# ECP-WarpX/WarpX

Hardware: AMD Instinct MI355X
Metric: particle_steps_per_s (higher is better)
Workload: dtype f64; 1 GPU; 3D uniform_plasma 256x256x256, 8 ppc, Yee FDTD, order-3 shape, esirkepov, boris, filter on; cells_per_gpu=16777216, particles_per_gpu=134217728, n_ranks=1, ranks_per_gpu=1, sort_interval=2, single_precision_comms=False, preroll_steps=40, overlap_halo=False, momentum_synchronisation=outside the timed region (the K steps are consecutive steps of one longer run)

## Files before the change

include/warpx_amd.h:

```cpp
#ifndef WARPX_AMD_H_
#define WARPX_AMD_H_

#include <stdint.h>

#ifdef __cplusplus
extern "C" {
#endif

typedef enum wxa_status {
    WXA_OK = 0,
    WXA_ERR_INVALID_ARG = -1,
    WXA_ERR_HIP = -2,
    WXA_ERR_UNSUPPORTED = -3,
    WXA_ERR_NOMEM = -4,
    WXA_ERR_COMM = -5
} wxa_status;

enum { WXA_PUSHER_BORIS = 0, WXA_PUSHER_VAY = 1, WXA_PUSHER_HC = 2,
       WXA_PUSHER_BORIS_RR = 3 };
enum { WXA_DEPOSIT_ESIRKEPOV = 0, WXA_DEPOSIT_DIRECT = 1 };
enum { WXA_DT_FULL = 0, WXA_DT_FIRST_HALF = 1, WXA_DT_SECOND_HALF = 2 };

typedef struct wxa_field_view {
    double* p;
// ... 168 lines not shown
                                    const int32_t sm_lo[3], const int32_t sm_hi[3], void* stream);

#define WXA_PBOUNDARY_DEFAULT    0
#define WXA_PBOUNDARY_ABSORBING  1
#define WXA_PBOUNDARY_REFLECTING 2
#define WXA_PBOUNDARY_PERIODIC   3

wxa_status wxa_apply_particle_boundaries(const wxa_particle_view* p, const double prob_lo[3],
                                         const double prob_hi[3], const int32_t bc_lo[3],
                                         const int32_t bc_hi[3], int64_t* n_lost,
                                         wxa_workspace* ws, void* stream);

wxa_status wxa_apply_pec_j(const wxa_field_view J[3], const int32_t dom_lo[3],
                           const int32_t dom_hi[3], const int32_t pec_lo[3],
                           const int32_t pec_hi[3], void* stream);

wxa_status wxa_apply_pec_rho(const wxa_field_view* rho, const int32_t dom_lo[3],
                             const int32_t dom_hi[3], const int32_t pec_lo[3],
                             const int32_t pec_hi[3], void* stream);


wxa_status wxa_filter_bilinear(const wxa_field_view* src, const wxa_field_view* dst,
                               void* stream);

wxa_status wxa_filter_stencil(const wxa_field_view* src, const wxa_field_view* dst, const double* s0, int32_t n0,
                              const double* s1, int32_t n1, const double* s2, int32_t n2, void* stream);

#define WXA_NCI_EX_EY_BZ 0
#define WXA_NCI_BX_BY_EZ 1
wxa_status wxa_nci_godfrey_stencil(double cdtodz, int32_t nodal_gather, int32_t coeff_set, double stencil_z[5]);

wxa_status wxa_fill_boundary_periodic(const wxa_field_view* f, const int ng[3],
                                      const int periodic[3], void* stream);

wxa_status wxa_fill_boundary_periodic_multi(const wxa_field_view* f, int32_t nf, const int ng[3],
                                            const int periodic[3], void* stream);

wxa_status wxa_sync_nodal_periodic(const wxa_field_view* f, const int periodic[3], void* stream);

wxa_status wxa_sum_boundary_periodic(const wxa_field_view* f, const int src_ng[3],
                                     const int periodic[3], void* stream);

wxa_status wxa_sum_boundary_periodic_multi(const wxa_field_view* f, int32_t nf, const int src_ng[3],
                                           const int periodic[3], void* stream);

wxa_status wxa_pack_box(const wxa_field_view* f, const int32_t blo[3], const int32_t bhi[3],
// ... 204 lines not shown
```

warpx_amd/_capi.py:

```python
from __future__ import annotations

import ctypes as C
import os

_HERE = os.path.dirname(os.path.abspath(__file__))
PRODUCT_LIB = os.path.join(_HERE, "libwarpx_amd.so")


class FieldView(C.Structure):
    _fields_ = [
        ("p", C.c_void_p),
        ("lo", C.c_int32 * 3),
        ("n", C.c_int32 * 3),
        ("ng", C.c_int32 * 3),
        ("stag", C.c_int32 * 3),
        ("jstride", C.c_int64),
        ("kstride", C.c_int64),
    ]


class ParticleView(C.Structure):
    _fields_ = [
        ("x", C.c_void_p), ("y", C.c_void_p), ("z", C.c_void_p), ("w", C.c_void_p),
        ("ux", C.c_void_p), ("uy", C.c_void_p), ("uz", C.c_void_p),
# ... 194 lines not shown
    "sim_get_field": (C.c_int, [C.c_void_p, C.c_char_p, _PFV]),
    "sim_get_particles": (C.c_int, [C.c_void_p, C.c_int32, _PPV]),
    "sim_get_timers": (C.c_int, [C.c_void_p, C.c_double * 8, C.c_int64 * 8, C.c_int]),
    "sim_enable_timers": (C.c_int, [C.c_void_p, C.c_int]),
    "sim_compute_rho": (C.c_int, [C.c_void_p]),
    "sim_halo_overlap": (C.c_int32, [C.c_void_p]),
    "sim_set_moving_window": (C.c_int, [C.c_void_p, C.POINTER(MovingWindow)]),
    "sim_set_injection": (C.c_int, [C.c_void_p, C.c_int32, C.POINTER(PlasmaInjector), C.c_int, C.c_int]),
    "sim_set_external_particle_fields": (C.c_int, [C.c_void_p, C.c_int32, _D3, _D3]),
    "sim_set_radiation_reaction": (C.c_int, [C.c_void_p, C.c_int32, C.c_int32]),
    "sim_add_laser": (C.c_int, [C.c_void_p, C.POINTER(LaserAntenna)]),
    "sim_add_btd": (C.c_int, [C.c_void_p, C.c_int32, C.c_double, C.c_int32, C.c_int32]),
    "sim_btd_num_particles": (C.c_int, [C.c_void_p, C.c_int32, C.c_int32, C.POINTER(C.c_int64)]),
    "sim_btd_particles": (C.c_int, [C.c_void_p, C.c_int32, C.c_int32, C.POINTER(C.c_double)]),
    "sim_btd_info": (C.c_int, [C.c_void_p, C.c_int32, C.POINTER(C.c_int32), C.POINTER(C.c_double), C.POINTER(C.c_double),
                              C.POINTER(C.c_int32), C.POINTER(C.c_int32)]),
    "sim_btd_data": (C.c_int, [C.c_void_p, C.c_int32, C.c_int32, C.POINTER(C.c_double)]),
    "sim_add_reduced_diag": (C.c_int, [C.c_void_p, C.c_char_p, C.c_char_p, C.c_char_p, C.c_char_p]),
    "sim_reduced_diag_data": (C.c_int, [C.c_void_p, C.c_char_p, C.c_int32, C.POINTER(C.c_double), C.c_int32,
                                       C.POINTER(C.c_int32)]),
}

_PRODUCT_SIGS = {
    "fill_boundary_periodic_multi": (C.c_int, [_PFV, C.c_int32, _I3, _I3, C.c_void_p]),
    "sum_boundary_periodic_multi": (C.c_int, [_PFV, C.c_int32, _I3, _I3, C.c_void_p]),
    "workspace_set_external_particle_fields": (C.c_int, [C.c_void_p, _D3, _D3]),
    "workspace_set_repeated_plasma_lens": (C.c_int, [C.c_void_p, C.POINTER(RepeatedPlasmaLens)]),
    "workspace_set_time": (C.c_int, [C.c_void_p, C.c_double]),
    "workspace_create": (C.c_int, [C.POINTER(C.c_void_p)]),
    "workspace_destroy": (None, [C.c_void_p]),
    "last_error": (C.c_char_p, []),
    "sort_particles_by_cell": (C.c_int, [_PPV, _PPV, _D3, _D3, _I32_3, _I32_3, C.c_void_p, C.c_void_p]),
    "gather_push_ws": (C.c_int, [_PPV, _FV3, _FV3, _PGG, C.c_double, C.c_double, C.c_double,
                                 C.c_int, C.c_int, C.c_int, C.c_int, C.c_void_p, C.c_void_p]),
    "add_plasma": (C.c_int, [_PPV, C.POINTER(PlasmaInjector), _D3, _I32_3, _D3, _D3, _D3,
                             C.POINTER(InjectedMomentum), C.POINTER(C.c_int64), C.c_void_p, C.c_void_p]),
    "gather_push_part": (C.c_int, [_PPV, _FV3, _FV3, _PGG, C.c_double, C.c_double, C.c_double, C.c_int, C.c_int,
                                   C.c_int, C.c_void_p, C.c_int, C.c_void_p]),
    "partition_particles": (C.c_int, [_PPV, _PPV, C.c_int, C.c_double, C.c_double,
                                      C.POINTER(C.c_int64), C.c_void_p, C.c_void_p]),
    "wrap_and_classify": (C.c_int, [_PPV, C.c_int64, C.c_int64, _D3, _D3, _I3, _D3, _D3, _I3, C.c_void_p,
                                    C.c_int64, C.POINTER(C.c_int64), C.c_void_p, C.c_void_p]),
    "wrap_and_classify_dest": (C.c_int, [_PPV, C.c_int64, C.c_int64, _D3, _D3, _I3, _D3, _D3, _I3, C.c_void_p,
                                         C.c_int64, C.POINTER(C.c_int64), C.c_void_p, C.c_void_p]),
    "pack_leavers": (C.c_int, [_PPV, C.c_void_p, C.c_int64, C.c_void_p, C.c_int64, C.c_int64, C.c_int, _D3, _D3,
                               C.c_void_p]),
# ... 176 lines not shown
```

warpx_amd/csrc/fields.hip:

```cpp
#include "common.hpp"

#include <algorithm>
#include <climits>
#include <cstdlib>

namespace wxa {

template <int TW_, int TJ_, int KC_, int NT_, int BATCH_ = 0>
struct StencilCfg {
    static constexpr int TW = TW_, TI = 64 * TW_, TJ = TJ_, KC = KC_, NT = NT_, BATCH = BATCH_;
};

struct TileGrid {
    int nti, ntj, ntk;
    long ntiles;
};

template <class CFG>
static TileGrid make_tiles_cfg(const Box3& ub) {
    TileGrid t;
    t.nti = (ub.hi[0] - ub.lo[0] + CFG::TI - 1) / CFG::TI;
    t.ntj = (ub.hi[1] - ub.lo[1] + CFG::TJ - 1) / CFG::TJ;
    t.ntk = (ub.hi[2] - ub.lo[2] + CFG::KC - 1) / CFG::KC;
    t.ntiles = (long)t.nti * t.ntj * t.ntk;
// ... 438 lines not shown
    DevF f[WXA_MULTI_MAX];
    BoxN lo[WXA_MULTI_MAX], hi[WXA_MULTI_MAX];
    int shift[WXA_MULTI_MAX];
};
__global__ void __launch_bounds__(256)
shift_copy_sides_multi_kernel(SideCopySet a, int d) {
    const int c = blockIdx.y;
    const DevF f = a.f[c];
    const BoxN box_lo = a.lo[c], box_hi = a.hi[c];
    const int s0 = d == 0 ? a.shift[c] : 0, s1 = d == 1 ? a.shift[c] : 0, s2 = d == 2 ? a.shift[c] : 0;
    const long half = (long)box_lo.n[0] * box_lo.n[1] * box_lo.n[2];
    for (long t = (long)blockIdx.x * blockDim.x + threadIdx.x; t < 2 * half; t += (long)gridDim.x * blockDim.x) {
        const bool hi = t >= half;
        const long u = hi ? t - half : t;
        const BoxN& box = hi ? box_hi : box_lo;
        const int sg = hi ? -1 : 1;
        const int aa = (int)(u % box.n[0]);
        const int bb = (int)((u / box.n[0]) % box.n[1]);
        const int cc = (int)(u / ((long)box.n[0] * box.n[1]));
        const int i = box.lo[0] + aa, j = box.lo[1] + bb, k = box.lo[2] + cc;
        f.p[f.off(i, j, k)] = f.p[f.off(i + sg * s0, j + sg * s1, k + sg * s2)];
    }
}
struct PeriodicSumSet {
    DevF f[WXA_MULTI_MAX];
    int nc[WXA_MULTI_MAX], s0[WXA_MULTI_MAX], s1[WXA_MULTI_MAX];
};
__global__ void __launch_bounds__(256)
sum_periodic_multi_kernel(PeriodicSumSet a, int d) {
    const int c = blockIdx.y;
    const DevF f = a.f[c];
    const int nc = a.nc[c], s0 = a.s0[c], s1 = a.s1[c];
    const int lo[3] = {f.lo0, f.lo1, f.lo2};
    const int n[3] = {f.n0, f.n1, f.n2};
    const long st[3] = {1, f.js, f.ks};
    const int da = d == 0 ? 1 : 0, db = d == 2 ? 1 : 2;
    const int nr = n[d] - nc;
    if (nr <= 0) return;
    const long total = (long)n[da] * nr * n[db];
    for (long t = (long)blockIdx.x * blockDim.x + threadIdx.x; t < total; t += (long)gridDim.x * blockDim.x) {
        int aa, r, b;
        if (d == 0) {
            r = (int)(t % nr); aa = (int)((t / nr) % n[da]); b = (int)(t / ((long)nr * n[da]));
        } else {
            aa = (int)(t % n[da]); r = (int)((t / n[da]) % nr); b = (int)(t / ((long)n[da] * nr));
        }
// ... 176 lines not shown
            double* b = &By(i, j, k);
            __builtin_nontemporal_store(__builtin_nontemporal_load(b) + (dt * ckc_up_x(ez, c.x, i, j, k) - dt * ckc_up_z(ex, c.z, i, j, k)), b);
        }
        if (pz && k >= bbz.lo[2] && k < bbz.hi[2]) {
            double* b = &Bz(i, j, k);
            __builtin_nontemporal_store(__builtin_nontemporal_load(b) + (dt * ckc_up_y(ex, c.y, i, j, k) - dt * ckc_up_x(ey, c.x, i, j, k)), b);
        }
        if constexpr (CFG::PIPE) {
            if (more) {
                ckc_put_plane<CFG>(ring[0] + ((k + 2) & 3) * PLANE, rx, tid);
                ckc_put_plane<CFG>(ring[1] + ((k + 2) & 3) * PLANE, ry, tid);
                ckc_put_plane<CFG>(ring[2] + ((k + 2) & 3) * PLANE, rz, tid);
            }
        }
        if constexpr (CFG::PIPE == 2) {
#pragma unroll
            for (int n = 0; n < CFG::PER; ++n) { rx[n] = qx[n]; ry[n] = qy[n]; rz[n] = qz[n]; }
        }
    }
}

using CkcProduction = CkcCfg<4, 16, 2>;
using FilterCfg = CkcCfg<8, 16, 1>;

struct FilterStencils {
    static constexpr int MAXLEN = 8;
    double s[3][MAXLEN];
    int n[3];
};
__global__ void __launch_bounds__(256)
filter_stencil_kernel(DevF src, DevF dst, FilterStencils fs) {
    const long total = (long)src.n0 * src.n1 * src.n2;
    for (long t = (long)blockIdx.x * blockDim.x + threadIdx.x; t < total; t += (long)gridDim.x * blockDim.x) {
        const int i = src.lo0 + (int)(t % src.n0);
        const int j = src.lo1 + (int)((t / src.n0) % src.n1);
        const int k = src.lo2 + (int)(t / ((long)src.n0 * src.n1));
        auto zp = [&](int ii, int jj, int kk) -> double {
            return (ii >= src.lo0 && ii < src.lo0 + src.n0 && jj >= src.lo1 && jj < src.lo1 + src.n1 && kk >= src.lo2 &&
                    kk < src.lo2 + src.n2) ? src.p[src.off(ii, jj, kk)] : 0.0;
        };
        double d = 0.0;
        for (int i2 = 0; i2 < fs.n[2]; ++i2)
            for (int i1 = 0; i1 < fs.n[1]; ++i1)
                for (int i0 = 0; i0 < fs.n[0]; ++i0) {
                    const double sss = fs.s[0][i0] * fs.s[1][i1] * fs.s[2][i2];
                    d += sss * (zp(i - i0, j - i1, k - i2) + zp(i + i0, j - i1, k - i2) + zp(i - i0, j + i1, k - i2) +
// ... 16 lines not shown
    const int k0 = src.lo2 + (int)(t / columns) * KC, k1 = min(k0 + KC, src.lo2 + src.n2);
    auto zp = [&](int kk) -> double { return (kk >= src.lo2 && kk < src.lo2 + src.n2) ? src.p[src.off(i, j, kk)] : 0.0; };
    double w[2 * N2 - 1];
#pragma unroll
    for (int m = 0; m < 2 * N2 - 1; ++m) w[m] = zp(k0 - (N2 - 1) + m);
    double sss[N2];
#pragma unroll
    for (int i2 = 0; i2 < N2; ++i2) sss[i2] = fs.s[0][0] * fs.s[1][0] * fs.s[2][i2];
    for (int k = k0; k < k1; ++k) {
        const double next = zp(k + N2);
        double d = 0.0;
#pragma unroll
        for (int i2 = 0; i2 < N2; ++i2) {
            const double a = w[N2 - 1 - i2], b = w[N2 - 1 + i2];
            d += sss[i2] * (a + a + a + a + b + b + b + b);
        }
        dst.p[dst.off(i, j, k)] = d;
#pragma unroll
        for (int m = 0; m + 1 < 2 * N2 - 1; ++m) w[m] = w[m + 1];
        w[2 * N2 - 2] = next;
    }
}

template <class CFG>
__global__ void __launch_bounds__(CFG::NT)
filter_bilinear_kernel(DevF src, DevF dst, TileGrid tg) {
    constexpr int PLANE = CFG::PLANE;
    __shared__ double ring[4 * PLANE];
    const long tile = xcd_tile_id(blockIdx.x, tg.ntiles);
    if (tile >= tg.ntiles) return;
    const int ti = (int)(tile % tg.nti), tj = (int)((tile / tg.nti) % tg.ntj), tk = (int)(tile / ((long)tg.nti * tg.ntj));
    const int i0 = src.lo0 + ti * CFG::TI, j0 = src.lo1 + tj * CFG::TJ, k0 = src.lo2 + tk * CFG::KC;
    const int hi0 = src.lo0 + src.n0, hi1 = src.lo1 + src.n1, hi2 = src.lo2 + src.n2;
    const int k1 = min(k0 + CFG::KC, hi2);
    const int tid = (int)(threadIdx.y * CFG::TI + threadIdx.x);
    const int i = i0 + (int)threadIdx.x, j = j0 + (int)threadIdx.y;
    double r[CFG::PER];
    for (int k = k0 - 1; k <= k0 + 1; ++k) {
        ckc_fetch_plane<CFG>(r, src, i0, j0, k, tid);
        ckc_put_plane<CFG>(ring + (k & 3) * PLANE, r, tid);
    }
    const CkcRing<CFG> in{ring, i0, j0};
    const bool active = i < hi0 && j < hi1;
    for (int k = k0; k < k1; ++k) {
        __syncthreads();
        const bool more = k + 2 <= k1;
        if (more) ckc_fetch_plane<CFG>(r, src, i0, j0, k + 2, tid);
        if (active) {
            auto tap = [&](int di, int dj, int dk) -> double { return in(i + di, j + dj, k + dk); };
            double d = 0.0;
#pragma unroll
            for (int i2 = 0; i2 < 2; ++i2)
#pragma unroll
                for (int i1 = 0; i1 < 2; ++i1)
#pragma unroll
                    for (int i0_ = 0; i0_ < 2; ++i0_) {
                        const double sss = 0.25 * 0.25 * 0.25;
                        d += sss * (tap(-i0_, -i1, -i2) + tap(+i0_, -i1, -i2) + tap(-i0_, +i1, -i2) +
                                    tap(+i0_, +i1, -i2) + tap(-i0_, -i1, +i2) + tap(+i0_, -i1, +i2) +
                                    tap(-i0_, +i1, +i2) + tap(+i0_, +i1, +i2));
                    }
            dst.p[dst.off(i, j, k)] = d;
        }
        if (more) ckc_put_plane<CFG>(ring + ((k + 2) & 3) * PLANE, r, tid);
    }
}

static inline int grid_for(long total, int block = 256, int cap = 256 * 16) {
    long g = (total + block - 1) / block;
    if (g < 1) g = 1;
    if (g > cap) g = cap;
    return (int)g;
}

static bool box_inside(const wxa_field_view& v, const int32_t blo[3], const int32_t bhi[3]) {
    for (int d = 0; d < 3; ++d)
        if (blo[d] < v.lo[d] || bhi[d] > v.lo[d] + v.n[d] || bhi[d] < blo[d]) return false;
    return true;
}

}

using namespace wxa;

extern "C" {

wxa_status wxa_evolve_b(const wxa_field_view E[3], const wxa_field_view B[3], double dt,
                        const double dinv[3], void* stream) {
// ... 181 lines not shown
    const Box3 bx = valid_box(E[0]), by = valid_box(E[1]), bz = valid_box(E[2]);
    for (int c = 0; c < 3; ++c) {
        const Box3 bj = valid_box(J[c]);
        const Box3 be = valid_box(E[c]);
        for (int d = 0; d < 3; ++d)
            WXA_REQUIRE(bj.lo[d] == be.lo[d] && bj.hi[d] == be.hi[d], "J and E valid boxes differ");
    }
    Box3 ub;
    for (int d = 0; d < 3; ++d) {
        ub.lo[d] = std::min(bx.lo[d], std::min(by.lo[d], bz.lo[d]));
        ub.hi[d] = std::max(bx.hi[d], std::max(by.hi[d], bz.hi[d]));
    }
    using CFG = StProduction;
    const TileGrid tg = make_tiles_cfg<CFG>(ub);
    if (tg.ntiles > 0)
        hipLaunchKernelGGL((evolve_e_kernel<CFG>), dim3((unsigned)xcd_grid_size(tg.ntiles)), dim3(CFG::TI, CFG::TJ), 0,
                           (hipStream_t)stream, make_devf(E[0]), make_devf(E[1]), make_devf(E[2]), make_devf(B[0]),
                           make_devf(B[1]), make_devf(B[2]), make_devf(J[0]), make_devf(J[1]), make_devf(J[2]), ub, bx, by, bz,
                           tg, dt, dinv[0], dinv[1], dinv[2]);
    WXA_LAUNCH_CHECK();
    return WXA_OK;
}

wxa_status wxa_filter_bilinear(const wxa_field_view* src, const wxa_field_view* dst, void* stream) {
    WXA_REQUIRE(src && dst && view_ok(*src) && view_ok(*dst), "bad field view");
    WXA_REQUIRE(src->p != dst->p, "src and dst must not alias");
    for (int d = 0; d < 3; ++d)
        WXA_REQUIRE(src->lo[d] == dst->lo[d] && src->n[d] == dst->n[d], "src/dst boxes differ");
    TileGrid tg;
    tg.nti = (src->n[0] + FilterCfg::TI - 1) / FilterCfg::TI;
    tg.ntj = (src->n[1] + FilterCfg::TJ - 1) / FilterCfg::TJ;
    tg.ntk = (src->n[2] + FilterCfg::KC - 1) / FilterCfg::KC;
    tg.ntiles = (long)tg.nti * tg.ntj * tg.ntk;
    hipLaunchKernelGGL(filter_bilinear_kernel<FilterCfg>, dim3((unsigned)xcd_grid_size(tg.ntiles)),
                       dim3(FilterCfg::TI, FilterCfg::TJ), 0, (hipStream_t)stream, make_devf(*src), make_devf(*dst), tg);
    WXA_LAUNCH_CHECK();
    return WXA_OK;
}

wxa_status wxa_filter_stencil(const wxa_field_view* src, const wxa_field_view* dst, const double* s0, int32_t n0,
                              const double* s1, int32_t n1, const double* s2, int32_t n2, void* stream) {
    WXA_REQUIRE(src && dst && view_ok(*src) && view_ok(*dst) && s0 && s1 && s2, "bad argument");
    WXA_REQUIRE(src->p != dst->p, "src and dst must not alias");
    WXA_REQUIRE(n0 >= 1 && n0 <= FilterStencils::MAXLEN && n1 >= 1 && n1 <= FilterStencils::MAXLEN && n2 >= 1 &&
                n2 <= FilterStencils::MAXLEN, "stencil length");
    for (int d = 0; d < 3; ++d)
        WXA_REQUIRE(src->lo[d] == dst->lo[d] && src->n[d] == dst->n[d], "src/dst boxes differ");
    FilterStencils fs;
    fs.n[0] = n0; fs.n[1] = n1; fs.n[2] = n2;
    for (int a = 0; a < FilterStencils::MAXLEN; ++a) {
        fs.s[0][a] = a < n0 ? s0[a] : 0.0; fs.s[1][a] = a < n1 ? s1[a] : 0.0; fs.s[2][a] = a < n2 ? s2[a] : 0.0;
    }
    const long total = (long)src->n[0] * src->n[1] * src->n[2];
    if (total == 0) return WXA_OK;
    if (n0 == 1 && n1 == 1 && n2 == 5) {
        constexpr int KC = 32;
        const long lanes = (long)src->n[0] * src->n[1] * ((src->n[2] + KC - 1) / KC);
        hipLaunchKernelGGL((filter_stencil_z_kernel<5, KC>), dim3((unsigned)((lanes + 255) / 256)), dim3(256), 0,
                           (hipStream_t)stream, make_devf(*src), make_devf(*dst), fs);
        WXA_LAUNCH_CHECK();
// ... 28 lines not shown
        sh[d] = nc;
        const long total = 2 * (long)blo.n[0] * blo.n[1] * blo.n[2];
        if (total > 0)
            hipLaunchKernelGGL(shift_copy_sides_kernel, dim3(grid_for(total)), dim3(256), 0, (hipStream_t)stream, df,
                               blo, bhi, sh[0], sh[1], sh[2]);
        lo[d] = v0 - ng[d];
        hi[d] = v1 + ng[d];
    }
    WXA_LAUNCH_CHECK();
    return WXA_OK;
}

wxa_status wxa_fill_boundary_periodic_multi(const wxa_field_view* f, int32_t nf, const int ng[3], const int periodic[3],
                                            void* stream) {
    WXA_REQUIRE(f && ng && periodic && nf >= 1 && nf <= WXA_MULTI_MAX, "bad argument");
    int lo[WXA_MULTI_MAX][3], hi[WXA_MULTI_MAX][3];
    for (int c = 0; c < nf; ++c) {
        WXA_REQUIRE(view_ok(f[c]), "bad field view");
        for (int d = 0; d < 3; ++d) {
            WXA_REQUIRE(ng[d] <= f[c].ng[d], "ng exceeds allocated guards");
            lo[c][d] = f[c].lo[d] + f[c].ng[d];
            hi[c][d] = f[c].lo[d] + f[c].n[d] - f[c].ng[d];
        }
    }
    for (int d = 0; d < 3; ++d) {
        if (!periodic[d] || ng[d] <= 0) continue;
        SideCopySet a;
        long most = 0;
        for (int c = 0; c < nf; ++c) {
            const int nc = f[c].n[d] - 2 * f[c].ng[d] - f[c].stag[d];
            WXA_REQUIRE(ng[d] <= nc, "guard depth exceeds the period");
            const int v0 = f[c].lo[d] + f[c].ng[d], v1 = f[c].lo[d] + f[c].n[d] - f[c].ng[d];
            a.f[c] = make_devf(f[c]);
            for (int e = 0; e < 3; ++e) { a.lo[c].lo[e] = a.hi[c].lo[e] = lo[c][e]; a.lo[c].n[e] = a.hi[c].n[e] = hi[c][e] - lo[c][e]; }
            a.lo[c].lo[d] = v0 - ng[d]; a.hi[c].lo[d] = v1;
            a.lo[c].n[d] = a.hi[c].n[d] = ng[d];
            a.shift[c] = nc;
            most = std::max(most, 2 * (long)a.lo[c].n[0] * a.lo[c].n[1] * a.lo[c].n[2]);
            lo[c][d] = v0 - ng[d];
            hi[c][d] = v1 + ng[d];
        }
        for (int c = nf; c < WXA_MULTI_MAX; ++c) { a.f[c] = a.f[0]; a.lo[c] = a.lo[0]; a.hi[c] = a.hi[0]; a.shift[c] = 0; }
        if (most > 0)
            hipLaunchKernelGGL(shift_copy_sides_multi_kernel, dim3(grid_for(most), (unsigned)nf), dim3(256), 0,
                               (hipStream_t)stream, a, d);
    }
// ... 304 lines not shown
```

warpx_amd/csrc/host/BrickComm.hpp:

```cpp
#ifndef WXA_HOST_BRICKCOMM_HPP_
#define WXA_HOST_BRICKCOMM_HPP_

#include "amrex_shim.hpp"

namespace wxa::host {

struct DeviceBuffer {
    const Backend* be = nullptr;
    void* p = nullptr;
    size_t cap = 0;
    void reserve(size_t bytes) {
        if (bytes <= cap) return;
        if (p) be->dfree(p);
        cap = bytes + bytes / 4 + 1024;
        p = be->dmalloc(cap);
        if (!p) throw std::runtime_error("DeviceBuffer: allocation failed");
    }
    ~DeviceBuffer() { if (p) be->dfree(p); }
};

struct Slabs {
    int32_t smlo[3], smhi[3], splo[3], sphi[3], rplo[3], rphi[3], rmlo[3], rmhi[3];
};

// ... 40 lines not shown
    void set_periodic(const int periodic[3]) {
        for (int d = 0; d < 3; ++d) m_periodic[d] = periodic[d] != 0;
    }
    bool periodic(int d) const { return m_periodic[d]; }
    bool has_neighbor(int d, int side) const {
        return m_periodic[d] || (side == 0 ? m_coord[d] > 0 : m_coord[d] < m_nb[d] - 1);
    }
    bool exchanges(int d) const { return m_nb[d] > 1; }
    int rank_of(const int c[3]) const { return c[0] + m_nb[0] * (c[1] + m_nb[1] * c[2]); }
    int neighbor(int d, int side) const {
        if (!has_neighbor(d, side)) return -1;
        int c[3] = {m_coord[0], m_coord[1], m_coord[2]};
        c[d] = (c[d] + (side ? 1 : -1) + m_nb[d]) % m_nb[d];
        return rank_of(c);
    }
    const int* nbricks() const { return m_nb; }
    const int* coord() const { return m_coord; }

    bool domain_face(int d, int side) const { return side == 0 ? m_coord[d] == 0 : m_coord[d] == m_nb[d] - 1; }
    bool reference_corners() const { return m_reference_corners; }
    void FillBoundary(const std::vector<amrex::MultiFab*>& mfs, const amrex::IntVect& ng, bool nodal_sync,
                      void* stream) {
        const size_t nf = mfs.size();
        std::vector<std::array<int, 3>> lo(nf), hi(nf);
        for (size_t c = 0; c < nf; ++c) {
            const wxa_field_view& f = mfs[c]->view();
            for (int d = 0; d < 3; ++d) {
                if (ng[d] > f.ng[d]) throw std::runtime_error("FillBoundary: ng exceeds allocated guard cells");
                lo[c][d] = f.lo[d] + f.ng[d];
                hi[c][d] = f.lo[d] + f.n[d] - f.ng[d];
                if (!m_periodic[d] && !reference_corners()) { lo[c][d] = f.lo[d]; hi[c][d] = f.lo[d] + f.n[d]; }
            }
        }
        for (int d = 0; d < 3; ++d) {
            if (!m_periodic[d] && !exchanges(d)) continue;
            if (self_periodic(d)) {
                if (!nodal_sync && ng[d] > 0 && m_be->fill_boundary_periodic_multi && nf >= 2 && nf <= 6) {
                    wxa_field_view v[6];
                    for (size_t c = 0; c < nf; ++c) v[c] = transverse_view(mfs[c]->view(), d, lo[c].data(), hi[c].data());
                    int per[3] = {0, 0, 0}, g[3] = {0, 0, 0};
                    per[d] = 1; g[d] = ng[d];
                    check(m_be->fill_boundary_periodic_multi(v, (int32_t)nf, g, per, stream));
                } else {
                    for (size_t c = 0; c < nf; ++c) {
                        const wxa_field_view& f = mfs[c]->view();
                        if (nodal_sync && f.stag[d]) self_op(f, d, 0, lo[c].data(), hi[c].data(), true, stream);
// ... 319 lines not shown
```

warpx_amd/csrc/host/WarpX.hpp:

```cpp
#ifndef WXA_HOST_WARPX_HPP_
#define WXA_HOST_WARPX_HPP_

#include <chrono>
#include <functional>

#include "BTDiagnostics.hpp"
#include "NCIGodfreyFilter.hpp"
#include "ReducedDiags.hpp"
#include "WarpXParticleContainer.hpp"

namespace wxa::host {

struct guardCellManager {
    amrex::IntVect ng_alloc_EB, ng_alloc_J, ng_depos_J, ng_FieldSolver, ng_FieldGather, ng_UpdateAux;

    void Init(const amrex::Real dt, const std::array<amrex::Real, 3>& dx, const int nox, const bool use_filter,
              const amrex::IntVect& bilinear_filter_stencil_length, const bool do_fdtd_nci_corr = false,
              const int nci_corr_stencil = 0, const bool safe_guard_cells = false) {
        constexpr double c = 299'792'458.;
        for (int d = 0; d < 3; ++d) {
            const int ng_tmp = nox;
            ng_alloc_EB[d] = (ng_tmp % 2) ? ng_tmp + 1 : ng_tmp;
            if (d == 2 && do_fdtd_nci_corr) {
                const int ng = ng_tmp + nci_corr_stencil;
// ... 438 lines not shown
        m_overlap = true;
    }
    bool halo_overlap() const { return m_overlap; }
    void order_streams(void* waiting_stream, int ev, void* recorded_stream) {
        if (!m_halo_events[ev]) return;
        m_be->event_record(m_halo_events[ev], recorded_stream);
        m_be->stream_wait_event(waiting_stream, m_halo_events[ev]);
    }

    void PushParticlesandDeposit(amrex::Real a_cur_time, bool skip_current = false,
                                 PushType push_type = PushType::Explicit) {
        if (m_eb_fill_in_flight) {
            mypc->PushInterior(m_fields, dt[0]);
            order_streams(m_ctx.stream, 3, m_comm_stream);
            m_eb_fill_in_flight = false;
        }
        mypc->Evolve(m_fields, 0, "current_fp", a_cur_time, dt[0], DtType::Full, skip_current, push_type);
    }

    void SyncCurrentAndRho() {
        PhaseTimer t(&m_ctx, kSyncCurrent);
        using warpx::fields::FieldType;
        auto J = m_fields.get_alldirs(FieldType::current_fp, 0);
        if (use_filter)
            for (int idim = 0; idim < 3; ++idim) ApplyFilterJ(J, 0, idim);
        if (m_overlap) {
            order_streams(m_comm_stream, 0, m_ctx.stream);
            SumBoundaryJ(J, 0, m_comm_stream);
            return;
        }
        SumBoundaryJ(J, 0);
        ApplyJfieldBoundary(0, J[0], J[1], J[2], PatchType::fine);
    }

    void ApplyJfieldBoundary(int , amrex::MultiFab* Jx, amrex::MultiFab* Jy, amrex::MultiFab* Jz,
                             PatchType ) {
        if (!m_pec_here) return;
        const wxa_field_view Jv[3] = {Jx->view(), Jy->view(), Jz->view()};
        if (m_be->apply_pec_j(Jv, m_dom_lo, m_dom_hi, m_pec_lo, m_pec_hi, m_ctx.stream) != 0)
            throw std::runtime_error("apply_pec_j failed");
    }

    amrex::MultiFab& ComputeRho() {
        if (!m_rho) {
            amrex::IntVect ng_rho;
            for (int d = 0; d < 3; ++d)
                ng_rho[d] = m_ctx.nox + 1 + static_cast<int>(std::ceil(299'792'458. * dt[0] / m_ctx.dx[d]));
            m_rho = std::make_unique<amrex::MultiFab>(m_be, m_ctx.brick_box, amrex::IntVect(1), ng_rho);
// ... 32 lines not shown
                    total += (size_t)(sl.hi[0] - sl.lo[0]) * (size_t)(sl.hi[1] - sl.lo[1]) * (size_t)(sl.hi[2] - sl.lo[2]);
                    slabs.push_back(sl);
                }
            }
        }
        if (total) {
            m_pec_rho_keep.be = m_be;
            m_pec_rho_keep.reserve(sizeof(double) * total);
            for (const Slab& sl : slabs)
                check(m_be->pack_box(&v, sl.lo, sl.hi, static_cast<double*>(m_pec_rho_keep.p) + sl.at, m_ctx.stream), "pack_box");
        }
        if (m_be->apply_pec_rho(&v, m_dom_lo, m_dom_hi, m_pec_lo, m_pec_hi, m_ctx.stream) != 0)
            throw std::runtime_error("apply_pec_rho failed");
        for (const Slab& sl : slabs)
            check(m_be->unpack_box(&v, sl.lo, sl.hi, static_cast<const double*>(m_pec_rho_keep.p) + sl.at,  0,
                                   m_ctx.stream), "unpack_box");
    }

    void ApplyFilterJ(const ablastr::fields::VectorField& current, int , int idim) {
        amrex::MultiFab& J = *current[idim];
        amrex::MultiFab& tmp = *m_filter_tmp[idim];
        check(m_be->filter_bilinear(&J.view(), &tmp.view(), m_ctx.stream), "filter_bilinear");
        J.swap_storage(tmp);
    }

    void SumBoundaryJ(const ablastr::fields::VectorField& current, int lev) { SumBoundaryJ(current, lev, m_ctx.stream); }
    void SumBoundaryJ(const ablastr::fields::VectorField& current, int , void* stream) {
        amrex::IntVect ng_depos_J = guard_cells.ng_depos_J;
        if (use_filter) ng_depos_J = ng_depos_J + amrex::IntVect(2) - amrex::IntVect(1);
        ng_depos_J = amrex::min(ng_depos_J, current[0]->nGrowVect());
        m_comm->SumBoundary({current[0], current[1], current[2]}, ng_depos_J, safe_guard_cells,
                            stream);
    }

    void DryComm(int reps, double ms[4]) {
        using warpx::fields::FieldType;
        reps = std::min(std::max(reps, 1), 64);
        auto J = m_fields.get_alldirs(FieldType::current_fp, 0);
        DeviceBuffer saved[3];
        for (int c = 0; c < 3; ++c) {
            const wxa_field_view v = J[c]->view();
            const size_t bytes = sizeof(double) * (size_t)v.kstride * (size_t)v.n[2];
            saved[c].be = m_be;
            saved[c].reserve(bytes);
            m_be->memcpy_async(saved[c].p, v.p, bytes, m_ctx.stream);
        }
// ... 200 lines not shown
```

warpx_amd/csrc/host/backend.hpp:

```cpp
#ifndef WXA_HOST_BACKEND_HPP_
#define WXA_HOST_BACKEND_HPP_

#include <cstddef>
#include <cstdint>

#include "../../../include/warpx_amd.h"

struct wxa_expr;

namespace wxa::host {

struct Backend {
    const char* name;
    int (*evolve_b)(const wxa_field_view*, const wxa_field_view*, double, const double*, void*);
    int (*evolve_e)(const wxa_field_view*, const wxa_field_view*, const wxa_field_view*, double,
                    const double*, void*);
    int (*evolve_b_guard_layer)(const wxa_field_view*, const wxa_field_view*, double, const double*, const int32_t* grow,
                                void*);
    void (*ckc_stencil_coefficients)(const double* cell_size, double* cx, double* cy, double* cz);
    double (*ckc_max_dt)(const double* cell_size);
    int (*evolve_b_ckc)(const wxa_field_view*, const wxa_field_view*, double, const double* cx, const double* cy,
                        const double* cz, void*);
    int (*ws_set_external_eb)(void* ws, const double* E, const double* B);
    int (*ws_set_repeated_plasma_lens)(void* ws, const wxa_repeated_plasma_lens*) = nullptr;
// ... 13 lines not shown
    int (*add_plasma_profile)(const wxa_particle_view* dst, const wxa_plasma_injector*, const double* corner,
                              const int32_t* ncells, const double* dx, const double* brick_lo, const double* brick_hi,
                              const wxa_injected_momentum* momentum, const wxa_expr* density,
                              const wxa_expr* const* momentum_exprs, double density_min, double density_max,
                              int64_t* n_added, void* ws, void*) = nullptr;
    int (*ws_set_injection_profile)(void* ws, const wxa_expr* density, const wxa_expr* const* momentum) = nullptr;
    const char* (*last_error)() = nullptr;
    int (*deposit_charge)(const wxa_particle_view*, const wxa_field_view*, const wxa_grid_geom*, double, int, void*);
    int (*apply_pec_e)(const wxa_field_view*, const int32_t* dom_lo, const int32_t* dom_hi, const int32_t* pec_lo,
                       const int32_t* pec_hi, const int32_t* ng, void*);
    int (*apply_pec_b)(const wxa_field_view*, const int32_t* dom_lo, const int32_t* dom_hi, const int32_t* pec_lo,
                       const int32_t* pec_hi, const int32_t* ng, void*);
    int (*apply_pec_j)(const wxa_field_view*, const int32_t* dom_lo, const int32_t* dom_hi, const int32_t* pec_lo,
                       const int32_t* pec_hi, void*);
    int (*apply_pec_rho)(const wxa_field_view*, const int32_t* dom_lo, const int32_t* dom_hi, const int32_t* pec_lo,
                         const int32_t* pec_hi, void*);
    int (*apply_silver_mueller)(const wxa_field_view* E, const wxa_field_view* B, double dt, const double* dinv,
                                const int32_t* dom_lo, const int32_t* dom_hi, const int32_t* sm_lo, const int32_t* sm_hi,
                                void*) = nullptr;
    int (*shift_field_window)(const wxa_field_view*, double* tmp, int32_t dir, int32_t num_shift, const int* periodic,
                              void*);
    int (*laser_push)(const wxa_particle_view*, const wxa_laser_push_params*, double t, double dt, void*);
    int (*filter_bilinear)(const wxa_field_view*, const wxa_field_view*, void*);
    int (*btd_select_particles)(const wxa_particle_view*, const double* const old6[6], double z_boost, double z_boost_old,
                                double t_boost, double dt, double t_lab, double gamma_boost, double* out, int64_t capacity,
                                int64_t* n_selected, void* stream) = nullptr;
    int (*reduce_field)(const wxa_field_view*, const int32_t* lo, const int32_t* hi, double* sum_sq, double* max_abs,
                        void* stream) = nullptr;
    int (*reduce_particles)(const wxa_particle_view*, double mass, int32_t photon, double* out6, void* stream) = nullptr;
    int (*filter_stencil)(const wxa_field_view*, const wxa_field_view*, const double* s0, int32_t n0, const double* s1,
                          int32_t n1, const double* s2, int32_t n2, void*) = nullptr;
    int (*fill_boundary_periodic)(const wxa_field_view*, const int*, const int*, void*);
    int (*sync_nodal_periodic)(const wxa_field_view*, const int*, void*);
    int (*sum_boundary_periodic)(const wxa_field_view*, const int*, const int*, void*);
    int (*fill_boundary_periodic_multi)(const wxa_field_view*, int32_t, const int*, const int*, void*) = nullptr;
    int (*sum_boundary_periodic_multi)(const wxa_field_view*, int32_t, const int*, const int*, void*) = nullptr;
    int (*pack_box)(const wxa_field_view*, const int32_t*, const int32_t*, double*, void*);
    int (*unpack_box)(const wxa_field_view*, const int32_t*, const int32_t*, const double*, int, void*);
    int (*pack_box_f32)(const wxa_field_view*, const int32_t*, const int32_t*, float*, void*) = nullptr;
    int (*unpack_box_f32)(const wxa_field_view*, const int32_t*, const int32_t*, const float*, int, void*) = nullptr;
    int (*field_set_zero)(const wxa_field_view*, void*);
    int (*field_set_zero_multi)(const wxa_field_view*, int32_t, void*) = nullptr;
    int (*enforce_periodic)(const wxa_particle_view*, const double*, const double*, const int*, void*);
    int (*enforce_periodic_sorted)(const wxa_particle_view*, const double*, const double*, const int*, void* ws, int32_t,
                                   void*) = nullptr;
    int (*sort_particles_by_cell)(const wxa_particle_view*, const wxa_particle_view*, const double*,
// ... 42 lines not shown
```

warpx_amd/csrc/host/warpx_host.hip:

```cpp
#include <hip/hip_runtime.h>

#include "../common.hpp"
#include "WarpXInputs.hpp"

namespace {

using wxa::host::Backend;

void* hip_dmalloc(size_t bytes) {
    void* p = nullptr;
    if (hipMalloc(&p, bytes ? bytes : 8) != hipSuccess) {
        wxa::set_last_error("hipMalloc of %zu bytes failed", bytes);
        return nullptr;
    }
    return p;
}
void hip_dfree(void* p) { if (p) (void)hipFree(p); }
int hip_memset_async(void* p, int v, size_t n, void* st) {
    return hipMemsetAsync(p, v, n, (hipStream_t)st) == hipSuccess ? 0 : WXA_ERR_HIP;
}
int hip_memcpy_async(void* d, const void* s, size_t n, void* st) {
    if (n == 0) return 0;
    return hipMemcpyAsync(d, s, n, hipMemcpyDeviceToDevice, (hipStream_t)st) == hipSuccess ? 0 : WXA_ERR_HIP;
}
// ... 64 lines not shown
                           const wxa_grid_geom* g, double q, double m, double dt, int o, int ga, int pu, int move,
                           void* ws, void* st) -> int {
            return wxa_gather_push_ws(p, E, B, g, q, m, dt, o, ga, pu, move, static_cast<wxa_workspace*>(ws), st); };
        b.gather_push_part = [](const wxa_particle_view* p, const wxa_field_view* E, const wxa_field_view* B,
                                const wxa_grid_geom* g, double q, double m, double dt, int o, int ga, int pu, void* ws,
                                int part, void* st) -> int {
            return wxa_gather_push_part(p, E, B, g, q, m, dt, o, ga, pu, static_cast<wxa_workspace*>(ws), part, st); };
        b.add_plasma = [](const wxa_particle_view* dst, const wxa_plasma_injector* inj, const double* corner,
                          const int32_t* nc, const double* dx, const double* blo, const double* bhi,
                          const wxa_injected_momentum* u, int64_t* n, void* ws, void* st) -> int {
            return wxa_add_plasma(dst, inj, corner, nc, dx, blo, bhi, u, n, static_cast<wxa_workspace*>(ws), st); };
        b.add_plasma_profile = [](const wxa_particle_view* dst, const wxa_plasma_injector* inj, const double* corner,
                                  const int32_t* nc, const double* dx, const double* blo, const double* bhi,
                                  const wxa_injected_momentum* u, const wxa_expr* dens, const wxa_expr* const* mom,
                                  double dmin, double dmax, int64_t* n, void* ws, void* st) -> int {
            return wxa_add_plasma_profile(dst, inj, corner, nc, dx, blo, bhi, u, dens, mom, dmin, dmax, n,
                                          static_cast<wxa_workspace*>(ws), st); };
        b.ws_set_injection_profile = [](void* ws, const wxa_expr* dens, const wxa_expr* const* mom) -> int {
            return wxa_workspace_set_injection_profile(static_cast<wxa_workspace*>(ws), dens, mom); };
        b.last_error = wxa_last_error;
        b.deposit_current = k_deposit;
        b.filter_bilinear = [](const wxa_field_view* s, const wxa_field_view* d, void* st) -> int {
            return wxa_filter_bilinear(s, d, st); };
        b.btd_select_particles = [](const wxa_particle_view* p, const double* const o[6], double zb, double zbo, double tb,
                                    double dt, double tl, double g, double* out, int64_t cap, int64_t* n, void* st) -> int {
            return wxa_btd_select_particles(p, o, zb, zbo, tb, dt, tl, g, out, cap, n, st); };
        b.reduce_field = [](const wxa_field_view* f, const int32_t* lo, const int32_t* hi, double* ss, double* mx,
                            void* st) -> int { return wxa_reduce_field(f, lo, hi, ss, mx, st); };
        b.reduce_particles = [](const wxa_particle_view* p, double m, int32_t photon, double* out, void* st) -> int {
            return wxa_reduce_particles(p, m, photon, out, st); };
        b.filter_stencil = [](const wxa_field_view* s, const wxa_field_view* d, const double* s0, int32_t n0,
                              const double* s1, int32_t n1, const double* s2, int32_t n2, void* st) -> int {
            return wxa_filter_stencil(s, d, s0, n0, s1, n1, s2, n2, st); };
        b.fill_boundary_periodic = [](const wxa_field_view* f, const int* ng, const int* per, void* st) -> int {
            return wxa_fill_boundary_periodic(f, ng, per, st); };
        b.sync_nodal_periodic = [](const wxa_field_view* f, const int* per, void* st) -> int {
            return wxa_sync_nodal_periodic(f, per, st); };
        b.sum_boundary_periodic = [](const wxa_field_view* f, const int* ng, const int* per, void* st) -> int {
            return wxa_sum_boundary_periodic(f, ng, per, st); };
        b.fill_boundary_periodic_multi = [](const wxa_field_view* f, int32_t nf, const int* ng, const int* per, void* st) -> int {
            return wxa_fill_boundary_periodic_multi(f, nf, ng, per, st); };
        b.sum_boundary_periodic_multi = [](const wxa_field_view* f, int32_t nf, const int* ng, const int* per, void* st) -> int {
            return wxa_sum_boundary_periodic_multi(f, nf, ng, per, st); };
        b.pack_box = [](const wxa_field_view* f, const int32_t* lo, const int32_t* hi, double* buf, void* st) -> int {
            return wxa_pack_box(f, lo, hi, buf, st); };
        b.unpack_box = [](const wxa_field_view* f, const int32_t* lo, const int32_t* hi, const double* buf, int mode,
// ... 125 lines not shown
```

Before: 11.16 billion particle-steps/s.

## Batch J filter into one launch, deepen prefetch, fuse periodic guard fill

Merges the three per-component bilinear current filters into a single multi-field kernel launch indexed by blockIdx.y. The filter now prefetches AHEAD planes into registers instead of one, to hide global load latency. Separately, periodic guard-cell fill across two or more directions becomes a single shell-copy kernel instead of sequential per-direction passes. This cuts launch count and serialization, at the cost of more registers per thread and an extra host-side fast path in FillBoundary.

```diff
diff --git a/include/warpx_amd.h b/include/warpx_amd.h
--- a/include/warpx_amd.h
+++ b/include/warpx_amd.h
@@ -214,6 +214,8 @@
 
 wxa_status wxa_filter_bilinear(const wxa_field_view* src, const wxa_field_view* dst,
                                void* stream);
+
+wxa_status wxa_filter_bilinear_multi(const wxa_field_view* src, const wxa_field_view* dst, int32_t nf, void* stream);
 
 wxa_status wxa_filter_stencil(const wxa_field_view* src, const wxa_field_view* dst, const double* s0, int32_t n0,
                               const double* s1, int32_t n1, const double* s2, int32_t n2, void* stream);
diff --git a/warpx_amd/_capi.py b/warpx_amd/_capi.py
--- a/warpx_amd/_capi.py
+++ b/warpx_amd/_capi.py
@@ -240,6 +240,7 @@
 }
 
 _PRODUCT_SIGS = {
+    "filter_bilinear_multi": (C.c_int, [_PFV, _PFV, C.c_int32, C.c_void_p]),
     "fill_boundary_periodic_multi": (C.c_int, [_PFV, C.c_int32, _I3, _I3, C.c_void_p]),
     "sum_boundary_periodic_multi": (C.c_int, [_PFV, C.c_int32, _I3, _I3, C.c_void_p]),
     "workspace_set_external_particle_fields": (C.c_int, [C.c_void_p, _D3, _D3]),
diff --git a/warpx_amd/csrc/fields.hip b/warpx_amd/csrc/fields.hip
--- a/warpx_amd/csrc/fields.hip
+++ b/warpx_amd/csrc/fields.hip
@@ -484,6 +484,41 @@
         f.p[f.off(i, j, k)] = f.p[f.off(i + sg * s0, j + sg * s1, k + sg * s2)];
     }
 }
+struct GuardShellSet {
+    DevF f[WXA_MULTI_MAX];
+    int v0[WXA_MULTI_MAX][3], v1[WXA_MULTI_MAX][3];
+    int nc[WXA_MULTI_MAX][3];
+    int g[3];
+};
+__global__ void __launch_bounds__(256)
+fill_guard_shell_multi_kernel(GuardShellSet a) {
+    const int c = blockIdx.y / 3, d = blockIdx.y % 3;
+    const int g = a.g[d];
+    if (g <= 0) return;
+    const DevF f = a.f[c];
+    int v0[3], v1[3], nc[3], lo[3], n[3];
+#pragma unroll
+    for (int e = 0; e < 3; ++e) {
+        v0[e] = a.v0[c][e]; v1[e] = a.v1[c][e]; nc[e] = a.nc[c][e];
+        const int ge = e < d ? a.g[e] : 0;
+        lo[e] = v0[e] - ge;
+        n[e] = v1[e] - v0[e] + 2 * ge;
+    }
+    n[d] = g;
+    const long half = (long)n[0] * n[1] * n[2];
+    for (long t = (long)blockIdx.x * blockDim.x + threadIdx.x; t < 2 * half; t += (long)gridDim.x * blockDim.x) {
+        const bool hi = t >= half;
+        const long u = hi ? t - half : t;
+        lo[d] = hi ? v1[d] : v0[d] - g;
+        int p[3], q[3];
+        p[0] = lo[0] + (int)(u % n[0]);
+        p[1] = lo[1] + (int)((u / n[0]) % n[1]);
+        p[2] = lo[2] + (int)(u / ((long)n[0] * n[1]));
+#pragma unroll
+        for (int e = 0; e < 3; ++e) q[e] = p[e] < v0[e] ? p[e] + nc[e] : p[e] >= v1[e] ? p[e] - nc[e] : p[e];
+        f.p[f.off(p[0], p[1], p[2])] = f.p[f.off(q[0], q[1], q[2])];
+    }
+}
 struct PeriodicSumSet {
     DevF f[WXA_MULTI_MAX];
     int nc[WXA_MULTI_MAX], s0[WXA_MULTI_MAX], s1[WXA_MULTI_MAX];
@@ -706,6 +741,9 @@
 
 using CkcProduction = CkcCfg<4, 16, 2>;
 using FilterCfg = CkcCfg<8, 16, 1>;
+#ifndef WXA_FILTER_AHEAD
+#define WXA_FILTER_AHEAD 2
+#endif
 
 struct FilterStencils {
     static constexpr int MAXLEN = 8;
@@ -768,31 +806,56 @@
     }
 }
 
+constexpr int WXA_FILTER_MAX = 3;
+struct FilterSet {
+    DevF src[WXA_FILTER_MAX], dst[WXA_FILTER_MAX];
+    TileGrid tg[WXA_FILTER_MAX];
+};
+__device__ double filter_zero = 0.0;
 template <class CFG>
+__device__ __forceinline__ void filter_fetch_plane(double (&r)[CFG::PER], const DevF& F, int i0, int j0, int kk, bool wanted,
+                                                   int tid) {
+    const bool kin = wanted && kk >= F.lo2 && kk < F.lo2 + F.n2;
+#pragma unroll
+    for (int n = 0; n < CFG::PER; ++n) {
+        const int a = tid + n * CFG::NT;
+        const int i = i0 - 1 + a % CFG::NI, j = j0 - 1 + a / CFG::NI;
+        const bool in = a < CFG::PLANE && kin && i >= F.lo0 && i < F.lo0 + F.n0 && j >= F.lo1 && j < F.lo1 + F.n1;
+        const double* from = in ? F.p + F.off(i, j, kk) : &filter_zero;
+        r[n] = *from;
+    }
+}
+template <class CFG, int AHEAD>
 __global__ void __launch_bounds__(CFG::NT)
-filter_bilinear_kernel(DevF src, DevF dst, TileGrid tg) {
+filter_bilinear_kernel(FilterSet fs) {
     constexpr int PLANE = CFG::PLANE;
     __shared__ double ring[4 * PLANE];
+    const int c = blockIdx.y;
+    const TileGrid tg = fs.tg[c];
     const long tile = xcd_tile_id(blockIdx.x, tg.ntiles);
     if (tile >= tg.ntiles) return;
+    const DevF src = fs.src[c], dst = fs.dst[c];
     const int ti = (int)(tile % tg.nti), tj = (int)((tile / tg.nti) % tg.ntj), tk = (int)(tile / ((long)tg.nti * tg.ntj));
     const int i0 = src.lo0 + ti * CFG::TI, j0 = src.lo1 + tj * CFG::TJ, k0 = src.lo2 + tk * CFG::KC;
     const int hi0 = src.lo0 + src.n0, hi1 = src.lo1 + src.n1, hi2 = src.lo2 + src.n2;
     const int k1 = min(k0 + CFG::KC, hi2);
     const int tid = (int)(threadIdx.y * CFG::TI + threadIdx.x);
-    const int i = i0 + (int)threadIdx.x, j = j0 + (int)threadIdx.y;
-    double r[CFG::PER];
+    const int i = min(i0 + (int)threadIdx.x, hi0 - 1), j = min(j0 + (int)threadIdx.y, hi1 - 1);
+    double q[AHEAD][CFG::PER];
     for (int k = k0 - 1; k <= k0 + 1; ++k) {
-        ckc_fetch_plane<CFG>(r, src, i0, j0, k, tid);
-        ckc_put_plane<CFG>(ring + (k & 3) * PLANE, r, tid);
-    }
+        filter_fetch_plane<CFG>(q[0], src, i0, j0, k, true, tid);
+        ckc_put_plane<CFG>(ring + (k & 3) * PLANE, q[0], tid);
+    }
+#pragma unroll
+    for (int s = 0; s + 1 < AHEAD; ++s) filter_fetch_plane<CFG>(q[s], src, i0, j0, k0 + 2 + s, k0 + 2 + s <= k1, tid);
     const CkcRing<CFG> in{ring, i0, j0};
-    const bool active = i < hi0 && j < hi1;
-    for (int k = k0; k < k1; ++k) {
-        __syncthreads();
-        const bool more = k + 2 <= k1;
-        if (more) ckc_fetch_plane<CFG>(r, src, i0, j0, k + 2, tid);
-        if (active) {
+    static_assert(CFG::KC % AHEAD == 0, "segments of whole groups");
+    auto group = [&](const int kb) {
+#pragma unroll
+        for (int s = 0; s < AHEAD; ++s) {
+            const int k = min(kb + s, k1 - 1);
+            __syncthreads();
+            filter_fetch_plane<CFG>(q[(s + AHEAD - 1) % AHEAD], src, i0, j0, kb + s + 1 + AHEAD, kb + s + 1 + AHEAD <= k1, tid);
             auto tap = [&](int di, int dj, int dk) -> double { return in(i + di, j + dj, k + dk); };
             double d = 0.0;
 #pragma unroll
@@ -807,9 +870,13 @@
                                     tap(-i0_, +i1, +i2) + tap(+i0_, +i1, +i2));
                     }
             dst.p[dst.off(i, j, k)] = d;
-        }
-        if (more) ckc_put_plane<CFG>(ring + ((k + 2) & 3) * PLANE, r, tid);
-    }
+#pragma unroll
+            for (int n = 0; n < CFG::PER; ++n) WXA_OPAQUE_F64(q[s][n]);
+            ckc_put_plane<CFG>(ring + ((k + 2) & 3) * PLANE, q[s], tid);
+        }
+    };
+    group(k0);
+    for (int kb = k0 + AHEAD; kb < k1; kb += AHEAD) group(kb);
 }
 
 static inline int grid_for(long total, int block = 256, int cap = 256 * 16) {
@@ -1037,20 +1104,35 @@
     return WXA_OK;
 }
 
+wxa_status wxa_filter_bilinear_multi(const wxa_field_view* src, const wxa_field_view* dst, int32_t nf, void* stream) {
+    WXA_REQUIRE(src && dst && nf >= 1 && nf <= WXA_FILTER_MAX, "bad argument");
+    FilterSet fs;
+    long most = 0;
+    for (int c = 0; c < nf; ++c) {
+        WXA_REQUIRE(view_ok(src[c]) && view_ok(dst[c]), "bad field view");
+        for (int e = 0; e < nf; ++e) WXA_REQUIRE(src[c].p != dst[e].p, "src and dst must not alias");
+        for (int d = 0; d < 3; ++d)
+            WXA_REQUIRE(src[c].lo[d] == dst[c].lo[d] && src[c].n[d] == dst[c].n[d], "src/dst boxes differ");
+        TileGrid& tg = fs.tg[c];
+        tg.nti = (src[c].n[0] + FilterCfg::TI - 1) / FilterCfg::TI;
+        tg.ntj = (src[c].n[1] + FilterCfg::TJ - 1) / FilterCfg::TJ;
+        tg.ntk = (src[c].n[2] + FilterCfg::KC - 1) / FilterCfg::KC;
+        tg.ntiles = (long)tg.nti * tg.ntj * tg.ntk;
+        fs.src[c] = make_devf(src[c]);
+        fs.dst[c] = make_devf(dst[c]);
+        most = std::max(most, tg.ntiles);
+    }
+    for (int c = nf; c < WXA_FILTER_MAX; ++c) { fs.src[c] = fs.src[0]; fs.dst[c] = fs.dst[0]; fs.tg[c] = fs.tg[0]; }
+    if (most > 0)
+        hipLaunchKernelGGL((filter_bilinear_kernel<FilterCfg, WXA_FILTER_AHEAD>), dim3((unsigned)xcd_grid_size(most), (unsigned)nf),
+                           dim3(FilterCfg::TI, FilterCfg::TJ), 0, (hipStream_t)stream, fs);
+    WXA_LAUNCH_CHECK();
+    return WXA_OK;
+}
+
 wxa_status wxa_filter_bilinear(const wxa_field_view* src, const wxa_field_view* dst, void* stream) {
-    WXA_REQUIRE(src && dst && view_ok(*src) && view_ok(*dst), "bad field view");
-    WXA_REQUIRE(src->p != dst->p, "src and dst must not alias");
-    for (int d = 0; d < 3; ++d)
-        WXA_REQUIRE(src->lo[d] == dst->lo[d] && src->n[d] == dst->n[d], "src/dst boxes differ");
-    TileGrid tg;
-    tg.nti = (src->n[0] + FilterCfg::TI - 1) / FilterCfg::TI;
-    tg.ntj = (src->n[1] + FilterCfg::TJ - 1) / FilterCfg::TJ;
-    tg.ntk = (src->n[2] + FilterCfg::KC - 1) / FilterCfg::KC;
-    tg.ntiles = (long)tg.nti * tg.ntj * tg.ntk;
-    hipLaunchKernelGGL(filter_bilinear_kernel<FilterCfg>, dim3((unsigned)xcd_grid_size(tg.ntiles)),
-                       dim3(FilterCfg::TI, FilterCfg::TJ), 0, (hipStream_t)stream, make_devf(*src), make_devf(*dst), tg);
-    WXA_LAUNCH_CHECK();
-    return WXA_OK;
+    WXA_REQUIRE(src && dst, "bad field view");
+    return wxa_filter_bilinear_multi(src, dst, 1, stream);
 }
 
 wxa_status wxa_filter_stencil(const wxa_field_view* src, const wxa_field_view* dst, const double* s0, int32_t n0,
@@ -1125,6 +1207,37 @@
             lo[c][d] = f[c].lo[d] + f[c].ng[d];
             hi[c][d] = f[c].lo[d] + f[c].n[d] - f[c].ng[d];
         }
+    }
+    int ndir = 0;
+    for (int d = 0; d < 3; ++d) ndir += periodic[d] && ng[d] > 0;
+    if (ndir >= 2) {
+        GuardShellSet a;
+        long most = 0;
+        for (int d = 0; d < 3; ++d) a.g[d] = periodic[d] && ng[d] > 0 ? ng[d] : 0;
+        for (int c = 0; c < nf; ++c) {
+            a.f[c] = make_devf(f[c]);
+            long pts[3];
+            for (int d = 0; d < 3; ++d) {
+                a.v0[c][d] = lo[c][d];
+                a.v1[c][d] = hi[c][d];
+                a.nc[c][d] = f[c].n[d] - 2 * f[c].ng[d] - f[c].stag[d];
+                WXA_REQUIRE(a.g[d] <= a.nc[c][d], "guard depth exceeds the period");
+                pts[d] = hi[c][d] - lo[c][d];
+            }
+            for (int d = 0; d < 3; ++d) {
+                if (a.g[d]) most = std::max(most, 2 * (long)a.g[d] * pts[(d + 1) % 3] * pts[(d + 2) % 3]);
+                pts[d] += 2 * a.g[d];
+            }
+        }
+        for (int c = nf; c < WXA_MULTI_MAX; ++c) {
+            a.f[c] = a.f[0];
+            for (int d = 0; d < 3; ++d) { a.v0[c][d] = a.v0[0][d]; a.v1[c][d] = a.v1[0][d]; a.nc[c][d] = a.nc[0][d]; }
+        }
+        if (most > 0)
+            hipLaunchKernelGGL(fill_guard_shell_multi_kernel, dim3(grid_for(most), (unsigned)(3 * nf)), dim3(256), 0,
+                               (hipStream_t)stream, a);
+        WXA_LAUNCH_CHECK();
+        return WXA_OK;
     }
     for (int d = 0; d < 3; ++d) {
         if (!periodic[d] || ng[d] <= 0) continue;
diff --git a/warpx_amd/csrc/host/BrickComm.hpp b/warpx_amd/csrc/host/BrickComm.hpp
--- a/warpx_amd/csrc/host/BrickComm.hpp
+++ b/warpx_amd/csrc/host/BrickComm.hpp
@@ -86,6 +86,23 @@
     void FillBoundary(const std::vector<amrex::MultiFab*>& mfs, const amrex::IntVect& ng, bool nodal_sync,
                       void* stream) {
         const size_t nf = mfs.size();
+        if (!nodal_sync && m_be->fill_boundary_periodic_multi && nf >= 2 && nf <= 6 && m_nb[0] == 1 && m_nb[1] == 1 &&
+            m_nb[2] == 1) {
+            int per[3], g[3], ndir = 0;
+            bool plain = true;
+            for (int d = 0; d < 3; ++d) {
+                per[d] = m_periodic[d] ? 1 : 0;
+                g[d] = m_periodic[d] ? ng[d] : 0;
+                ndir += per[d] && g[d] > 0;
+                plain = plain && (m_periodic[d] || reference_corners());
+            }
+            if (plain && ndir >= 2) {
+                wxa_field_view v[6];
+                for (size_t c = 0; c < nf; ++c) v[c] = mfs[c]->view();
+                check(m_be->fill_boundary_periodic_multi(v, (int32_t)nf, g, per, stream));
+                return;
+            }
+        }
         std::vector<std::array<int, 3>> lo(nf), hi(nf);
         for (size_t c = 0; c < nf; ++c) {
             const wxa_field_view& f = mfs[c]->view();
diff --git a/warpx_amd/csrc/host/WarpX.hpp b/warpx_amd/csrc/host/WarpX.hpp
--- a/warpx_amd/csrc/host/WarpX.hpp
+++ b/warpx_amd/csrc/host/WarpX.hpp
@@ -484,8 +484,7 @@
         PhaseTimer t(&m_ctx, kSyncCurrent);
         using warpx::fields::FieldType;
         auto J = m_fields.get_alldirs(FieldType::current_fp, 0);
-        if (use_filter)
-            for (int idim = 0; idim < 3; ++idim) ApplyFilterJ(J, 0, idim);
+        if (use_filter) ApplyFilterJ(J, 0);
         if (m_overlap) {
             order_streams(m_comm_stream, 0, m_ctx.stream);
             SumBoundaryJ(J, 0, m_comm_stream);
@@ -564,6 +563,16 @@
         amrex::MultiFab& tmp = *m_filter_tmp[idim];
         check(m_be->filter_bilinear(&J.view(), &tmp.view(), m_ctx.stream), "filter_bilinear");
         J.swap_storage(tmp);
+    }
+    void ApplyFilterJ(const ablastr::fields::VectorField& current, int lev) {
+        if (!m_be->filter_bilinear_multi) {
+            for (int idim = 0; idim < 3; ++idim) ApplyFilterJ(current, lev, idim);
+            return;
+        }
+        const wxa_field_view src[3] = {current[0]->view(), current[1]->view(), current[2]->view()};
+        const wxa_field_view dst[3] = {m_filter_tmp[0]->view(), m_filter_tmp[1]->view(), m_filter_tmp[2]->view()};
+        check(m_be->filter_bilinear_multi(src, dst, 3, m_ctx.stream), "filter_bilinear_multi");
+        for (int idim = 0; idim < 3; ++idim) current[idim]->swap_storage(*m_filter_tmp[idim]);
     }
 
     void SumBoundaryJ(const ablastr::fields::VectorField& current, int lev) { SumBoundaryJ(current, lev, m_ctx.stream); }
diff --git a/warpx_amd/csrc/host/backend.hpp b/warpx_amd/csrc/host/backend.hpp
--- a/warpx_amd/csrc/host/backend.hpp
+++ b/warpx_amd/csrc/host/backend.hpp
@@ -59,6 +59,7 @@
                               void*);
     int (*laser_push)(const wxa_particle_view*, const wxa_laser_push_params*, double t, double dt, void*);
     int (*filter_bilinear)(const wxa_field_view*, const wxa_field_view*, void*);
+    int (*filter_bilinear_multi)(const wxa_field_view*, const wxa_field_view*, int32_t, void*) = nullptr;
     int (*btd_select_particles)(const wxa_particle_view*, const double* const old6[6], double z_boost, double z_boost_old,
                                 double t_boost, double dt, double t_lab, double gamma_boost, double* out, int64_t capacity,
                                 int64_t* n_selected, void* stream) = nullptr;
diff --git a/warpx_amd/csrc/host/warpx_host.hip b/warpx_amd/csrc/host/warpx_host.hip
--- a/warpx_amd/csrc/host/warpx_host.hip
+++ b/warpx_amd/csrc/host/warpx_host.hip
@@ -110,6 +110,8 @@
         b.deposit_current = k_deposit;
         b.filter_bilinear = [](const wxa_field_view* s, const wxa_field_view* d, void* st) -> int {
             return wxa_filter_bilinear(s, d, st); };
+        b.filter_bilinear_multi = [](const wxa_field_view* s, const wxa_field_view* d, int32_t nf, void* st) -> int {
+            return wxa_filter_bilinear_multi(s, d, nf, st); };
         b.btd_select_particles = [](const wxa_particle_view* p, const double* const o[6], double zb, double zbo, double tb,
                                     double dt, double tl, double g, double* out, int64_t cap, int64_t* n, void* st) -> int {
             return wxa_btd_select_particles(p, o, zb, zbo, tb, dt, tl, g, out, cap, n, st); };
```

Measured after the change: 10.91 billion particle-steps/s. 0.977x the previous value.
